# EnterpriseCV-6/Season-NeRF

Measured on AMD Instinct MI355X. Metric: ray-samples/sec (4096 rays x 96 samples forward render, T_NeRF 8x256), higher is better.
Workload: dtype i8x3 (16-bit fixed point as two int8 digits on v_mfma_i32_32x32x32_i8, exact int32 accumulate, fp32 epilogue)

## Files before the change

season_nerf_amd/csrc/kernels_i8x2.hip:

```cpp
#include "mlp_i8_device.h"

namespace snerf {

constexpr int NW2 = 8;
constexpr int TILE2 = 32 * NW2;
constexpr int PIECES2 = kChunkBytes / kFragBytes / NW2;
constexpr int RING2_D = 7;
#ifndef SNERF_PFX
#define SNERF_PFX 2
#endif
constexpr int PFX = SNERF_PFX;
static_assert(PIECES2 == 2 && kChunkPairs == 8, "the DMA below moves two pieces per wave; barrier positions assume 8-pair chunks");

#ifdef SNERF_STAMP
__device__ unsigned long long g_stamps[8 * 64];
__device__ __forceinline__ void stamp(int wave, int lane, int slot, bool on) {
    if (on && lane == 0) g_stamps[wave * 64 + slot] = __builtin_amdgcn_s_memtime();
}
#define STAMP(slot) stamp(wave, lane, slot, stamp_on)
#else
#define STAMP(slot)
#endif

struct Ring2 {
    uint32_t wr;
    uint32_t goff;
    uint32_t cur;
};
__device__ __forceinline__ uint32_t ring2_next(uint32_t off) {
    off += kChunkBytes;
    return off == RING2_D * kChunkBytes ? 0u : off;
}
__device__ __forceinline__ void dma_chunk2(const uint8_t* stream, uint32_t goff, lds_char* lds, uint32_t wr, int wave, int lane);
__device__ __forceinline__ void dma_chunk4(const uint8_t* stream, uint32_t goff, lds_char* lds, uint32_t wr, int wave, int lane);
#ifndef SNERF_X2_ALL_LOAD
#define SNERF_X2_OLD_LOADS 1
#endif
template <int PHASE>
__device__ __forceinline__ void ring_step2(Ring2& rg, const uint8_t* stream, uint32_t stream_bytes, lds_char* lds, int wave, int lane) {
#if defined(SNERF_ABLATE) && (ABL & 4)
    return;
#endif
#if defined(SNERF_X2_OLD_LOADS) && !defined(SNERF_STAMP)
    if (PHASE == 0) {
        asm volatile("s_waitcnt vmcnt(%0)\n\ts_barrier" ::"n"((RING2_D - 3) * 4) : "memory");
        dma_chunk4(stream, rg.goff, lds, rg.wr, wave, lane);
    } else {
        asm volatile("s_barrier" ::: "memory");
    }
    rg.goff += kChunkBytes;
    if (rg.goff >= stream_bytes) rg.goff = 0;
    rg.wr = ring2_next(rg.wr);
    return;
#endif
#ifdef SNERF_STAMP
    const unsigned long long t0_ = __builtin_amdgcn_s_memtime();
    asm volatile("s_waitcnt vmcnt(%0)" ::"n"((RING2_D - 3) * PIECES2) : "memory");
    const unsigned long long t1_ = __builtin_amdgcn_s_memtime();
    asm volatile("s_barrier" ::: "memory");
    const unsigned long long t2_ = __builtin_amdgcn_s_memtime();
    if (blockIdx.x == 0 && lane == 0) { g_stamps[wave * 64 + 62] += t1_ - t0_; g_stamps[wave * 64 + 63] += t2_ - t1_; }
#else
    asm volatile("s_waitcnt vmcnt(%0)\n\ts_barrier" ::"n"((RING2_D - 3) * PIECES2) : "memory");
#endif
    dma_chunk2(stream, rg.goff, lds, rg.wr, wave, lane);
    rg.goff += kChunkBytes;
    if (rg.goff >= stream_bytes) rg.goff = 0;
    rg.wr = ring2_next(rg.wr);
}
__device__ __forceinline__ void dma_chunk2(const uint8_t* stream, uint32_t goff, lds_char* lds, uint32_t wr, int wave, int lane) {
    const uint8_t* b0 = stream + goff + wave * (PIECES2 * kFragBytes);
    const uint32_t dst = (uint32_t)(uintptr_t)(lds + wr + wave * (PIECES2 * kFragBytes));
    const uint32_t voff = lane * 16;
    uint32_t keep;
    asm volatile(
        "s_mov_b32 %0, m0\n\t"
        "s_mov_b32 m0, %2\n\t"
        "s_nop 0\n\t"
        "global_load_lds_dwordx4 %1, %3\n\t"
        "s_add_u32 m0, m0, 0x400\n\t"
        "s_nop 0\n\t"
        "global_load_lds_dwordx4 %1, %4\n\t"
        "s_mov_b32 m0, %0"
        : "=&s"(keep)
        : "v"(voff), "s"(dst), "s"(b0), "s"(b0 + kFragBytes)
        : "memory", "scc");
}

__device__ __forceinline__ void dma_chunk4(const uint8_t* stream, uint32_t goff, lds_char* lds, uint32_t wr, int wave, int lane) {
    const uint8_t* b0 = stream + goff + wave * (4 * kFragBytes);
    const uint32_t dst = (uint32_t)(uintptr_t)(lds + wr + wave * (4 * kFragBytes));
    const uint32_t voff = lane * 16;
    uint32_t keep;
    asm volatile(
        "s_mov_b32 %0, m0\n\t"
        "s_mov_b32 m0, %2\n\t"
        "s_nop 0\n\t"
        "global_load_lds_dwordx4 %1, %3\n\t"
        "s_add_u32 m0, m0, 0x400\n\t"
        "s_nop 0\n\t"
        "global_load_lds_dwordx4 %1, %4\n\t"
        "s_add_u32 m0, m0, 0x400\n\t"
        "s_nop 0\n\t"
        "global_load_lds_dwordx4 %1, %5\n\t"
        "s_add_u32 m0, m0, 0x400\n\t"
        "s_nop 0\n\t"
        "global_load_lds_dwordx4 %1, %6\n\t"
        "s_mov_b32 m0, %0"
        : "=&s"(keep)
        : "v"(voff), "s"(dst), "s"(b0), "s"(b0 + kFragBytes), "s"(b0 + 2 * kFragBytes), "s"(b0 + 3 * kFragBytes)
        : "memory", "scc");
}

struct TabQ {
    f32x4 sc, bi;
};
__device__ __forceinline__ TabQ load_tab_quad(lds_cfloat* tab_l, int b, int h, int g) {
    typedef volatile const __attribute__((address_space(3))) f32x4 lds_vf32x4;
    lds_vf32x4* tp = (lds_vf32x4*)(tab_l + (b * 2 + h) * 32);
    TabQ t;
    t.sc = tp[g];
    t.bi = tp[4 + g];
    return t;
}
__device__ __forceinline__ TabQ load_tab_quad_h(lds_cfloat* tab_h, int b, int g) {
    typedef volatile const __attribute__((address_space(3))) f32x4 lds_vf32x4;
    lds_vf32x4* tp = (lds_vf32x4*)(tab_h + b * 64);
    TabQ t;
    t.sc = tp[g];
    t.bi = tp[4 + g];
    return t;
}
template <int NB, int KS0, int KS1, bool SIN, bool RAWL = false, int PHASE = 0, bool OPQ = false>
__device__ __forceinline__ void run_layer8x2(Ring2& rg, const uint8_t* stream, uint32_t stream_bytes, lds_char* lds, lds_cfloat* tab_l,
                                             const Frag8* in0, const Frag8* in1, Frag8* out, f32x16* raw, int wave, int lane,
                                             const float* rawx = nullptr) {
    constexpr int KS = KS0 + KS1, NP = NB * KS;
    typedef volatile const __attribute__((address_space(3))) f32x4 lds_vf32x4;
    f32x4 rq[4][3];
    const int h = lane >> 5;
    lds_cfloat* raw_l = tab_l + 2 * 32 * NB;
    lds_cfloat* tab_h = tab_l + 32 * h;
    lds_cfloat* raw_h = raw_l + 48 * h;
    if constexpr (OPQ) asm volatile("" : "+v"(tab_h), "+v"(raw_h));
    auto tabq = [&](int b_, int g_) { return OPQ ? load_tab_quad_h(tab_h, b_, g_) : load_tab_quad(tab_l, b_, h, g_); };
    i32x4 fT[PFX], fL[PFX];
#if defined(SNERF_ABLATE) && (ABL & 2)
    constexpr bool ABL2_ = true;
#pragma unroll
    for (int q = 0; q < PFX; ++q) { fT[q] = i32x4{lane, 1, 2, 3}; fL[q] = i32x4{4, lane, 6, 7}; }
#else
    constexpr bool ABL2_ = false;
#endif
#define REQUEST(QN, SLOT)                                                                              \
    do {                                                                                               \
        if ((QN) % kChunkPairs == 0) {                                                                 \
            ring_step2<PHASE>(rg, stream, stream_bytes, lds, wave, lane);                                \
            if ((QN) > 0) rg.cur = ring2_next(rg.cur);                                                 \
        }                                                                                              \
        lds_char* ap_ = lds + rg.cur + ((QN) % kChunkPairs) * kPairBytes + lane * 16;                  \
        if (!ABL2_) {                                                                                  \
            fT[SLOT] = *(lds_ci32x4*)ap_;                                                              \
            fL[SLOT] = *(lds_ci32x4*)(ap_ + kFragBytes);                                               \
        } else {                                                                                       \
            asm volatile("" : "+v"(fT[SLOT]), "+v"(fL[SLOT]));                                         \
        }                                                                                              \
    } while (0)
#pragma unroll
    for (int q = 0; q < PFX; ++q) {
        if (q < NP) REQUEST(q, q);
    }
    Acc8 acc;
    int m[16];
    TabQ tq[4];
    auto load_rq = [&](int g, int b_of) {
        if constexpr (RAWL) {
            lds_vf32x4* tp = OPQ ? (lds_vf32x4*)(raw_h + (b_of * 8 + g) * 12) : (lds_vf32x4*)(raw_l + ((b_of * 2 + h) * 4 + g) * 12);
            rq[g][0] = tp[0]; rq[g][1] = tp[1]; rq[g][2] = tp[2];
        }
    };
    auto quad = [&](int g, int b_of, const TabQ& t) {
        float v[4];
#pragma unroll
        for (int j = 0; j < 4; ++j) v[j] = __builtin_fmaf((float)m[4 * g + j], t.sc[j], t.bi[j]);
        if constexpr (RAWL) {
#pragma unroll
            for (int j = 0; j < 4; ++j)
                v[j] = __builtin_fmaf(rq[g][0][j], rawx[0], __builtin_fmaf(rq[g][1][j], rawx[1], __builtin_fmaf(rq[g][2][j], rawx[2], v[j])));
        }
        if (SIN) {
            int hi, lo;
            digits4(sin2pi(v[0]), sin2pi(v[1]), sin2pi(v[2]), sin2pi(v[3]), hi, lo);
            asm volatile("" : "+v"(hi), "+v"(lo));
            out[b_of].hi[g] = hi;
            out[b_of].lo[g] = lo;
        } else {
#pragma unroll
            for (int j = 0; j < 4; ++j) (*raw)[4 * g + j] = v[j];
        }
    };
#pragma unroll
    for (int b = 0; b < NB; ++b) {
        if (b > 0) {
            tq[0] = tabq(b - 1, 0);
            load_rq(0, b - 1);
#pragma unroll
            for (int i = 0; i < 16; ++i) m[i] = (int)(((uint32_t)acc.M[i] << 8) + (uint32_t)acc.X[i]);
            asm volatile("" ::: "memory");
            __builtin_amdgcn_sched_barrier(0);
        }
#pragma unroll
        for (int i = 0; i < 16; ++i) { acc.M[i] = 0; acc.X[i] = 0; }
#pragma unroll
        for (int s = 0; s < KS; ++s) {
            const int q = b * KS + s;
            const i32x4 aT = fT[q % PFX], aL = fL[q % PFX];
#ifndef SNERF_X2_NOPRIO
            if (((s + PHASE) & 1) == 0) __builtin_amdgcn_s_setprio(0); else __builtin_amdgcn_s_setprio(3);
#endif
            if (q + PFX < NP) REQUEST(q + PFX, q % PFX);
            if (b > 0) {
#pragma unroll
                for (int g = 1; g < 4; ++g) {
                    const int sg = (g * KS) / 4, lg = sg > 0 ? sg - 1 : 0;
                    if (lg == s) { tq[g] = tabq(b - 1, g); load_rq(g, b - 1); }
                }
            }
            mfma_i8x3(aT, aL, s < KS0 ? in0[s] : in1[s - KS0], acc);
            if (b > 0) {
#pragma unroll
                for (int g = 0; g < 4; ++g)
                    if ((g * KS) / 4 == s) quad(g, b - 1, tq[g]);
            }
            asm volatile("" ::: "memory");
#ifdef SNERF_X2_GROUPS
#pragma unroll
            for (int mm = 0; mm < 3; ++mm) {
                __builtin_amdgcn_sched_group_barrier(0x008, 1, 0);
                __builtin_amdgcn_sched_group_barrier(0x100, 1, 0);
                __builtin_amdgcn_sched_group_barrier(0x400, 2, 0);
                __builtin_amdgcn_sched_group_barrier(0x002, SNERF_X2_GROUPS, 0);
            }
#endif
            __builtin_amdgcn_sched_barrier(0);
        }
    }
#pragma unroll
    for (int i = 0; i < 16; ++i) m[i] = (int)(((uint32_t)acc.M[i] << 8) + (uint32_t)acc.X[i]);
#pragma unroll
    for (int g = 0; g < 4; ++g) {
        asm volatile("" ::: "memory");
        const TabQ t = tabq(NB - 1, g);
        load_rq(g, NB - 1);
        quad(g, NB - 1, t);
        asm volatile("" ::: "memory");
        __builtin_amdgcn_sched_barrier(0);
    }
    rg.cur = ring2_next(rg.cur);
#undef REQUEST
}

template <int W, int VARIANT, int PHASE>
__device__ __forceinline__ void field_tiles2(const MlpArgs& A, Ring2& rg, lds_char* lds, __attribute__((address_space(3))) float* tab_lds,
                                             int wave, int lane);

template <int W, int VARIANT>
__global__ __launch_bounds__(64 * NW2, 1) void mlp_i8x2_kernel(const MlpArgs A) {
    extern __shared__ __attribute__((aligned(16))) char smem[];
    constexpr int C_MAX = kMaxClasses;
    constexpr int W2 = W / 2;
    lds_char* lds = (lds_char*)smem;
    __attribute__((address_space(3))) float* tab_lds = (__attribute__((address_space(3))) float*)(lds + RING2_D * kChunkBytes);

    const int lane = threadIdx.x & 63;
    const int wave = __builtin_amdgcn_readfirstlane(threadIdx.x >> 6);
    const int h = lane >> 5;
    const int C = A.n_classes;

    for (int i = threadIdx.x; i < A.bias_floats; i += 64 * NW2) tab_lds[i] = A.bias[i];

    Ring2 rg;
    rg.cur = 0;
    rg.goff = 0;
    {
        uint32_t wr = 0;
#pragma unroll
        for (int c = 0; c < RING2_D - 2; ++c) {
#if defined(SNERF_X2_OLD_LOADS) && !defined(SNERF_STAMP)
            if (wave < 4) dma_chunk4(A.stream, rg.goff, lds, wr, wave, lane);
#else
            dma_chunk2(A.stream, rg.goff, lds, wr, wave, lane);
#endif
            rg.goff += kChunkBytes;
            if (rg.goff >= A.stream_bytes) rg.goff = 0;
            wr += kChunkBytes;
        }
        rg.wr = wr;
    }
    __syncthreads();

    if (wave < 4) field_tiles2<W, VARIANT, 0>(A, rg, lds, tab_lds, wave, lane);
    else field_tiles2<W, VARIANT, 1>(A, rg, lds, tab_lds, wave, lane);
    asm volatile("s_waitcnt vmcnt(0)" ::: "memory");
}

template <int W, int VARIANT, int PHASE>
__device__ __forceinline__ void field_tiles2(const MlpArgs& A, Ring2& rg, lds_char* lds, __attribute__((address_space(3))) float* tab_lds,
                                             int wave, int lane) {
    constexpr int C_MAX = kMaxClasses;
    constexpr int W2 = W / 2;
    const int h = lane >> 5;
    const int C = A.n_classes;
    const int64_t n_tiles = VARIANT == 3 ? (A.n + NW2 - 1) / NW2 : (A.n + TILE2 - 1) / TILE2;
    const int passes = VARIANT == 3 ? (A.n_samples + 31) / 32 : 1;
    int pass = 0;
    RaySum rs;
    for (int64_t tile = blockIdx.x; tile < n_tiles;) {
        const int64_t n = tile * TILE2 + wave * 32 + (lane & 31);
        const bool valid = n < A.n;
        const int64_t nc = valid ? n : A.n - 1;
        const int64_t g = VARIANT == 3 ? 0 : nc / A.group_size;

        float x0, x1, x2;
        if constexpr (VARIANT == 3) {
            raysum_point(rs, A, tile, NW2, wave, pass, lane, x0, x1, x2);
        } else if (A.points) {
            x0 = A.points[nc * 3]; x1 = A.points[nc * 3 + 1]; x2 = A.points[nc * 3 + 2];
        } else {
            const int64_t r = nc / A.n_samples;
            const int s = (int)(nc - r * A.n_samples);
            const float t = A.tvals[s], omt = __fsub_rn(1.f, t);
            x0 = __fadd_rn(__fmul_rn(A.top[r * 3], omt), __fmul_rn(A.bot[r * 3], t));
            x1 = __fadd_rn(__fmul_rn(A.top[r * 3 + 1], omt), __fmul_rn(A.bot[r * 3 + 1], t));
            x2 = __fadd_rn(__fmul_rn(A.top[r * 3 + 2], omt), __fmul_rn(A.bot[r * 3 + 2], t));
        }
        float s0 = 0.f, s1 = 0.f, s2 = 0.f;
        float pcls[C_MAX];
#pragma unroll
        for (int c = 0; c < C_MAX; ++c) pcls[c] = 0.f;
        if constexpr (VARIANT <= 1) { s0 = A.sun[g * 3]; s1 = A.sun[g * 3 + 1]; s2 = A.sun[g * 3 + 2]; }
        if constexpr (VARIANT == 0) {
            if (A.classes) {
#pragma unroll
                for (int c = 0; c < C_MAX; ++c) if (c < C) pcls[c] = A.classes[g * C + c];
            }
        }
#ifdef SNERF_STAMP
        const bool stamp_on = blockIdx.x == 0 && tile == (int64_t)blockIdx.x + gridDim.x;
#endif
        STAMP(0);
        Frag8 pe[PEPOS_KS8];
        make_pe_pos8<VARIANT == 3>(x0, x1, x2, h, pe);
        STAMP(1);

        constexpr int KW = W / 32, KW2 = W2 / 32;
        Frag8 hA[KW], hB[KW];
        f32x16 raw;
#define LAYER(L, NBv, K0, K1, SINv, IN0, IN1, OUT, RAW)                                                                       \
    run_layer8x2<NBv, K0, K1, SINv, false, PHASE, VARIANT == 3>(rg, A.stream, A.stream_bytes, lds, tab_lds + prog_table_start(PROG_FIELD, W, C_MAX, L), \
                                                  IN0, IN1, OUT, RAW, wave, lane)
#define LAYER_RAW(L, NBv, K0, K1, IN0, IN1, OUT, RX)                                                                          \
    run_layer8x2<NBv, K0, K1, true, true, PHASE, VARIANT == 3>(rg, A.stream, A.stream_bytes, lds, tab_lds + prog_table_start(PROG_FIELD, W, C_MAX, L), \
                                                 IN0, IN1, OUT, nullptr, wave, lane, RX)
        const float rx_p[3] = {x0, x1, x2}, rx_s[3] = {s0, s1, s2};
        LAYER_RAW(F_FC1, W / 32, PEPOS_KS8, 0, pe, nullptr, hA, rx_p); STAMP(2);
        LAYER(F_FC2, W / 32, KW, 0, true, hA, nullptr, hB, nullptr); STAMP(3);
        LAYER(F_FC3, W / 32, KW, 0, true, hB, nullptr, hA, nullptr); STAMP(4);
        LAYER(F_FC4, W / 32, KW, 0, true, hA, nullptr, hB, nullptr); STAMP(5);
        LAYER_RAW(F_FC5, W / 32, KW, PEPOS_KS8, hB, pe, hA, rx_p); STAMP(6);
        LAYER(F_FC6, W / 32, KW, 0, true, hA, nullptr, hB, nullptr); STAMP(7);
        LAYER(F_FC7, W / 32, KW, 0, true, hB, nullptr, hA, nullptr); STAMP(8);
        LAYER(F_FC8, W / 32, KW, 0, true, hA, nullptr, hB, nullptr); STAMP(9);
        Frag8 x1f[KW2];
        LAYER(F_FC9, W2 / 32, KW, 0, true, hB, nullptr, x1f, nullptr); STAMP(10);
        LAYER(F_HEAD, 1, KW2, 0, false, x1f, nullptr, nullptr, &raw); STAMP(11);
        const float col_r = raw[0], col_g = raw[1], col_b = raw[2], rho_raw = raw[3];
        float sv_raw = 0.f;
        float adj[3 * C_MAX];
#pragma unroll
        for (int i = 0; i < 3 * C_MAX; ++i) adj[i] = 0.f;
        if constexpr (VARIANT <= 1) {
            Frag8 ps[PESUN_KS8];
            make_pe_sun8(s0, s1, s2, h, ps);
            Frag8 sA[KW2], sB[KW2];
            LAYER_RAW(F_S1, W2 / 32, KW2, PESUN_KS8, x1f, ps, sA, rx_s); STAMP(12);
            LAYER(F_S2, W2 / 32, KW2, 0, true, sA, nullptr, sB, nullptr); STAMP(13);
            LAYER(F_S3, W2 / 32, KW2, 0, true, sB, nullptr, sA, nullptr); STAMP(14);
            LAYER(F_S4, 1, KW2, 0, false, sA, nullptr, nullptr, &raw); STAMP(15);
            sv_raw = raw[0];
        }
        if constexpr (VARIANT == 0) {
            LAYER(F_A1, W / 32, KW2, 0, true, x1f, nullptr, hA, nullptr); STAMP(16);
            LAYER(F_A2, W / 32, KW, 0, true, hA, nullptr, hB, nullptr); STAMP(17);
            LAYER(F_A3, W / 32, KW, 0, true, hB, nullptr, hA, nullptr); STAMP(18);
            LAYER(F_AC, 1, KW, 0, false, hA, nullptr, nullptr, &raw); STAMP(19);
#pragma unroll
            for (int i = 0; i < 3 * C_MAX; ++i) adj[i] = raw[i];
        }
#undef LAYER
#undef LAYER_RAW
        if constexpr (VARIANT == 3) {
            raysum_add(rs, A, tile, NW2, wave, pass, lane, rho_raw, x0, x1, x2);
            if (++pass == passes || raysum_saturated(rs, A, tile * NW2 + wave, wave, NW2, lane, (__attribute__((address_space(3))) float*)(tab_lds + A.bias_floats))) {
                raysum_end(rs, A, tile, NW2, wave, lane);
                pass = 0;
                tile += gridDim.x;
            }
        } else {
            if (h == 0 && valid) store_field_outputs<VARIANT>(A.out, n, C, x0, x1, x2, col_r, col_g, col_b, rho_raw, sv_raw, adj, pcls);
            tile += gridDim.x;
        }
        STAMP(20);
    }
    __builtin_amdgcn_s_setprio(0);
}

template <int W, int VARIANT>
static hipError_t launch_mlp_i8x2_t(const MlpArgs& a, int n_cu, hipStream_t st) {
    const int lds_bytes = RING2_D * kChunkBytes + a.bias_floats * 4 + kVoteBytes;
    const int64_t n_tiles = VARIANT == 3 ? (a.n + NW2 - 1) / NW2 : (a.n + TILE2 - 1) / TILE2;
    int grid = (int)(n_tiles < n_cu ? n_tiles : n_cu);
    if (grid < 1) grid = 1;
    auto k = mlp_i8x2_kernel<W, VARIANT>;
    hipError_t e = hipFuncSetAttribute((const void*)k, hipFuncAttributeMaxDynamicSharedMemorySize, lds_bytes);
    if (e != hipSuccess) return e;
    hipLaunchKernelGGL(k, dim3(grid), dim3(64 * NW2), lds_bytes, st, a);
    return hipGetLastError();
}

hipError_t launch_mlp_i8x2(int W, int variant, const MlpArgs& a, int n_cu, hipStream_t st) {
#define CASE(Wv)                                                              \
    if (W == Wv) {                                                            \
        if (variant == 0) return launch_mlp_i8x2_t<Wv, 0>(a, n_cu, st);       \
        if (variant == 1) return launch_mlp_i8x2_t<Wv, 1>(a, n_cu, st);       \
        if (variant == 3) return launch_mlp_i8x2_t<Wv, 3>(a, n_cu, st);       \
        return launch_mlp_i8x2_t<Wv, 2>(a, n_cu, st);                         \
    }
    CASE(64)
    CASE(256)
#undef CASE
    return hipErrorInvalidValue;
}

}

#ifdef SNERF_STAMP
extern "C" int snerf_debug_stamps(unsigned long long* host, int n) {
    if (n > 8 * 64) n = 8 * 64;
    hipError_t e = hipMemcpyFromSymbol(host, HIP_SYMBOL(snerf::g_stamps), (size_t)n * 8);
    unsigned long long zero[8 * 64] = {};
    (void)hipMemcpyToSymbol(HIP_SYMBOL(snerf::g_stamps), zero, sizeof(zero));
    return e == hipSuccess ? 0 : -3;
}
#endif
```

season_nerf_amd/csrc/pack.cpp:

```cpp
#include <atomic>
#include <cstdlib>
#include <mutex>
#include <thread>
#include "pack.h"

#include <cmath>
#include <cstring>

namespace snerf {

template <class F>
static bool parallel_layers(int L, std::string* err, F fn) {
    static const int cap = [] {
        const char* e = getenv("SNERF_PACK_THREADS");
        const unsigned hw = std::thread::hardware_concurrency();
        const int c = e ? atoi(e) : (int)(hw ? (hw < 8 ? hw : 8) : 1);
        return c < 1 ? 1 : c;
    }();
    const int T = cap < L ? cap : L;
    std::atomic<int> next{0};
    std::atomic<bool> ok{true};
    std::mutex mu;
    auto work = [&]() {
        for (;;) {
            const int l = next.fetch_add(1);
            if (l >= L || !ok.load()) break;
            std::string e;
            bool good = false;
            try {
                good = fn(l, &e);
            } catch (const std::exception& ex) {
                e = std::string("packing layer ") + std::to_string(l) + ": " + ex.what();
            } catch (...) {
                e = "packing layer " + std::to_string(l) + ": unknown exception";
            }
            if (!good) {
                std::lock_guard<std::mutex> g(mu);
                if (ok.exchange(false)) *err = e;
            }
        }
    };
    std::vector<std::thread> th;
    for (int t = 1; t < T; ++t) th.emplace_back(work);
    work();
    for (auto& t : th) t.join();
    return ok.load();
}

static inline uint16_t bf16_rne(float f) {
    uint32_t u;
    std::memcpy(&u, &f, 4);
    if ((u & 0x7f800000u) == 0x7f800000u) return (uint16_t)(u >> 16);
    u += 0x7fffu + ((u >> 16) & 1u);
    return (uint16_t)(u >> 16);
}
static inline float bf16_to_f32(uint16_t b) {
    uint32_t u = (uint32_t)b << 16;
    float f;
    std::memcpy(&f, &u, 4);
    return f;
}

const Tensor* Weights::find(const std::string& k) const {
    auto it = t.find(k);
    return it == t.end() ? nullptr : &it->second;
}

struct Src {
    const char* prefix;
    bool sine;
};

static const char* field_prefix(int l) {
    static const char* p[F_NUM] = {
        "G_NeRF_net.fc1", "G_NeRF_net.fc2", "G_NeRF_net.fc3", "G_NeRF_net.fc4", "G_NeRF_net.fc5", "G_NeRF_net.fc6",
        "G_NeRF_net.fc7", "G_NeRF_net.fc8", "G_NeRF_net.fc9", nullptr ,
        "G_NeRF_net.fc_solar_1", "G_NeRF_net.fc_solar_2", "G_NeRF_net.fc_solar_3", "G_NeRF_net.fc_solar_4",
        "adjust_layer_1", "adjust_layer_2", "adjust_layer_3", "adjust_col"};
    return p[l];
}
static const char* group_prefix(int l) {
    static const char* p[G_NUM] = {"time_layer_1", "time_layer_2", "get_class_layer", "G_NeRF_net.fc_sky_color_1",
                                   "G_NeRF_net.fc_sky_color_2"};
    return p[l];
}

struct Dense {
    int n = 0, k = 0;
    std::vector<double> W, b;
};

static bool fetch(const Weights& w, const std::string& key, size_t numel, const float** out, std::string* err) {
    const Tensor* t = w.find(key);
    if (!t) { *err = "missing tensor: " + key; return false; }
    if (t->data.size() != numel) {
        *err = "tensor " + key + " has " + std::to_string(t->data.size()) + " elements, expected " + std::to_string(numel);
        return false;
    }
    *out = t->data.data();
    return true;
}

static bool dense_sine(const Weights& w, const std::string& pre, int n, int k, bool fold_bn, Dense* d, std::string* err) {
    const float *W, *b;
    if (!fetch(w, pre + ".linear.weight", (size_t)n * k, &W, err)) return false;
    if (!fetch(w, pre + ".linear.bias", (size_t)n, &b, err)) return false;
    const bool has_bn = w.find(pre + ".norm.weight") != nullptr;
    const float *g = nullptr, *beta = nullptr, *mu = nullptr, *var = nullptr;
    if (has_bn) {
        if (!fold_bn) { *err = "layer " + pre + " has BatchNorm; only the folded (eval-mode) program is packed"; return false; }
        if (!fetch(w, pre + ".norm.weight", n, &g, err) || !fetch(w, pre + ".norm.bias", n, &beta, err) ||
            !fetch(w, pre + ".norm.running_mean", n, &mu, err) || !fetch(w, pre + ".norm.running_var", n, &var, err))
            return false;
    }
    const double inv2pi = 1.0 / (2.0 * M_PI);
    d->n = n; d->k = k;
    d->W.assign((size_t)n * k, 0.0); d->b.assign(n, 0.0);
    for (int r = 0; r < n; ++r) {
        double a = 1.0, shift = 0.0, off = 0.0;
        if (has_bn) { a = (double)g[r] / std::sqrt((double)var[r] + 1e-5); shift = mu[r]; off = beta[r]; }
        for (int c = 0; c < k; ++c) d->W[(size_t)r * k + c] = a * 30.0 * (double)W[(size_t)r * k + c] * inv2pi;
        d->b[r] = (a * (30.0 * (double)b[r] - shift) + off) * inv2pi;
    }
    return true;
}

static bool dense_linear(const Weights& w, const std::string& pre, int n, int k, Dense* d, std::string* err) {
    const float *W, *b;
    if (!fetch(w, pre + ".weight", (size_t)n * k, &W, err)) return false;
    if (!fetch(w, pre + ".bias", (size_t)n, &b, err)) return false;
    d->n = n; d->k = k;
    d->W.assign(W, W + (size_t)n * k);
    d->b.assign(b, b + n);
    return true;
}

static int ref_row(const LayerShape& s, int n) {
    const int b = n / 32, r = n % 32;
    switch (s.row_map) {
        case ROWS_ID: return n < s.n_ref ? n : -1;
        case ROWS_HEAD: return (b == 0 && r < 4) ? r : -1;
        case ROWS_SV: case ROWS_SKY: return (b == 0 && r < s.n_ref) ? r : -1;
        case ROWS_ADJ: case ROWS_CLASS:
            if (b != 0) return -1;
            for (int i = 0; i < s.n_ref && i < 16; ++i) if (acc_row(i, 0) == r) return i;
            return -1;
    }
    return -1;
}

static bool dense_layer(const Weights& w, int prog, int W, int C, int l, bool fold_bn, Dense* dp, std::string* err) {
    Dense& d = *dp;
    const LayerShape s = prog_layer(prog, W, C, l);
    const int k_ref = kind_features(s.kind0, s.ks0) + kind_features(s.kind1, s.ks1);
    if (prog == PROG_FIELD && l == F_HEAD) {
        Dense c3, s1;
        if (!dense_linear(w, "G_NeRF_net.fc10Col", 3, k_ref, &c3, err)) return false;
        if (!dense_linear(w, "G_NeRF_net.fc10Sigma", 1, k_ref, &s1, err)) return false;
        d.n = 4; d.k = k_ref; d.W = c3.W; d.b = c3.b;
        d.W.insert(d.W.end(), s1.W.begin(), s1.W.end()); d.b.push_back(s1.b[0]);
    } else {
        const std::string pre = prog == PROG_FIELD ? field_prefix(l) : group_prefix(l);
        int kr = k_ref;
        if (prog == PROG_GROUP && l == G_K2) kr = W / 4;
        if (s.out_kind == OUT_SIN) { if (!dense_sine(w, pre, s.n_ref, kr, fold_bn, &d, err)) return false; }
        else { if (!dense_linear(w, pre, s.n_ref, kr, &d, err)) return false; }
    }
    return true;
}

bool pack_program(const Weights& w, int prog, int W, int C, bool fold_bn, Packed* out, std::string* err) {
    if (W < 64 || W % 64 != 0) { *err = "layer width must be a multiple of 64 (got " + std::to_string(W) + ")"; return false; }
    if (C < 1 || C > kMaxClasses) { *err = "n_classes must be in [1," + std::to_string(kMaxClasses) + "]"; return false; }
    const int L = prog_layers(prog);
    out->stream.assign((size_t)prog_chunks(prog, W, C) * kChunkBytes, 0);
    out->bias.assign((size_t)prog_bias_floats(prog, W, C), 0.f);
    return parallel_layers(L, err, [&](int l, std::string* err) {
        const LayerShape s = prog_layer(prog, W, C, l);
        Dense d;
        if (!dense_layer(w, prog, W, C, l, fold_bn, &d, err)) return false;
        float* bias = out->bias.data() + prog_bias_start(prog, W, C, l);
        for (int b = 0; b < s.nb(); ++b)
            for (int h = 0; h < 2; ++h)
                for (int i = 0; i < 16; ++i) {
                    const int rr = ref_row(s, 32 * b + acc_row(i, h));
                    bias[b * 32 + h * 16 + i] = rr >= 0 ? (float)d.b[rr] : 0.f;
                }
        uint8_t* base = out->stream.data() + (size_t)prog_chunk_start(prog, W, C, l) * kChunkBytes;
        const int f0 = kind_features(s.kind0, s.ks0);
        for (int b = 0; b < s.nb(); ++b)
            for (int ks = 0; ks < s.ks(); ++ks) {
                uint16_t* hi = (uint16_t*)(base + (size_t)(b * s.ks() + ks) * kPairBytes);
                uint16_t* lo = hi + kFragBytes / 2;
                for (int lane = 0; lane < 64; ++lane) {
                    const int r = lane & 31, h = lane >> 5;
                    const int rr = ref_row(s, 32 * b + r);
                    for (int j = 0; j < 8; ++j) {
                        double v = 0.0;
                        if (rr >= 0) {
                            int col = -1;
                            if (ks < s.ks0) { const int f = slot_feature(s.kind0, 16 * ks + 8 * h + j); if (f >= 0) col = f; }
                            else { const int f = slot_feature(s.kind1, 16 * (ks - s.ks0) + 8 * h + j); if (f >= 0) col = f0 + f; }
                            if (col >= 0 && col < d.k) v = d.W[(size_t)rr * d.k + col];
                        }
                        const float vf = (float)v;
                        const uint16_t vh = bf16_rne(vf);
                        hi[lane * 8 + j] = vh;
                        lo[lane * 8 + j] = bf16_rne((float)(v - (double)bf16_to_f32(vh)));
                    }
                }
            }
        return true;
    });
}

bool permute_program_ks(const Packed& canon, int W, int C, Packed* out, std::string* err, int prog) {
    if (W % 256 != 0) { *err = "the K-split kernels need a width that is a multiple of 256 (got " + std::to_string(W) + ")"; return false; }
    if (canon.stream.size() != (size_t)prog_chunks(prog, W, C) * kChunkBytes) { *err = "permute_program_ks: not a packed program of this kind and width"; return false; }
    const int L = prog_layers(prog);
    auto start = [&](int l) { return prog == PROG_FIELD ? ks_chunk_start(W, C, l) : ks_chunk_start_g(W, C, l); };
    out->bias = canon.bias;
    out->stream.assign((size_t)start(L) * kChunkBytes, 0);
    for (int l = 0; l < L; ++l) {
        const LayerShape s = prog_layer(prog, W, C, l);
        const uint8_t* src = canon.stream.data() + (size_t)prog_chunk_start(prog, W, C, l) * kChunkBytes;
        uint8_t* dst = out->stream.data() + (size_t)start(l) * kChunkBytes;
        const int np = ks_layer_pairs(s);
        for (int a = 0; a < 2; ++a)
            for (int q = 0; q < np; ++q) {
                const int sp = ks_pair_source(s, a, q), b = sp / 4096, ks = sp % 4096;
                std::memcpy(dst + (size_t)(q / kKsParPairs) * kChunkBytes + (size_t)a * kKsParPairs * kPairBytes + (size_t)(q % kKsParPairs) * kPairBytes,
                            src + (size_t)(b * s.ks() + ks) * kPairBytes, kPairBytes);
            }
    }
    return true;
}

bool pack_program_i8(const Weights& w, int prog, int W, int C, bool fold_bn, Packed* out, std::string* err) {
    if (W < 64 || W % 64 != 0) { *err = "layer width must be a multiple of 64 (got " + std::to_string(W) + ")"; return false; }
    if (C < 1 || C > kMaxClasses) { *err = "n_classes must be in [1," + std::to_string(kMaxClasses) + "]"; return false; }
    const int L = prog_layers(prog);
    out->stream.assign((size_t)prog_chunks(prog, W, C, FMT_I8) * kChunkBytes, 0);
    out->bias.assign((size_t)prog_table_floats(prog, W, C), 0.f);
    return parallel_layers(L, err, [&](int l, std::string* err) {
        const LayerShape s = prog_layer(prog, W, C, l, FMT_I8);
        Dense d;
        if (!dense_layer(w, prog, W, C, l, fold_bn, &d, err)) return false;
        const int f0 = kind_features(s.kind0, s.ks0, FMT_I8);
        auto column = [&](int ks, int h, int j) {
            int col = -1;
            if (ks < s.ks0) { const int f = slot_feature8(s.kind0, ks, h, j); if (f >= 0) col = f; }
            else { const int f = slot_feature8(s.kind1, ks - s.ks0, h, j); if (f >= 0) col = f0 + f; }
            return (col >= 0 && col < d.k) ? col : -1;
        };
        const int rk = raw_kind(s), rdims = raw_dims(rk), rbase = (rk != IN_NONE && rk == s.kind1 && rk != s.kind0) ? f0 : 0;
        auto is_raw_col = [&](int c) { return rk != IN_NONE && c >= rbase && c < rbase + rdims; };
        const int n_pad = s.n_out;
        std::vector<double> scale(n_pad, 0.0);
        std::vector<long long> wsum(n_pad, 0);
        std::vector<int> wq((size_t)n_pad * d.k, 0);
        for (int n = 0; n < n_pad; ++n) {
            const int rr = ref_row(s, n);
            if (rr < 0) continue;
            double mx = 0.0;
            for (int c = 0; c < d.k; ++c) if (!is_raw_col(c)) mx = std::fmax(mx, std::fabs(d.W[(size_t)rr * d.k + c]));
            const double sn = mx > 0.0 ? mx / 32512.0 : 1.0;
            scale[n] = sn;
            for (int c = 0; c < d.k; ++c) wq[(size_t)n * d.k + c] = (int)std::llround(d.W[(size_t)rr * d.k + c] / sn);
        }
        uint8_t* base = out->stream.data() + (size_t)prog_chunk_start(prog, W, C, l, FMT_I8) * kChunkBytes;
        for (int b = 0; b < s.nb(); ++b)
            for (int ks = 0; ks < s.ks(); ++ks) {
                int8_t* Tf = (int8_t*)(base + (size_t)(b * s.ks() + ks) * kPairBytes);
                int8_t* Lf = Tf + kFragBytes;
                for (int lane = 0; lane < 64; ++lane) {
                    const int r = lane & 31, h = lane >> 5, n = 32 * b + r;
                    for (int j = 0; j < 16; ++j) {
                        const int col = column(ks, h, j);
                        int q = 0;
                        if (col >= 0 && ref_row(s, n) >= 0) { q = wq[(size_t)n * d.k + col]; wsum[n] += q; }
                        const int T = (q + 128) >> 8;
                        Tf[lane * 16 + j] = (int8_t)T;
                        Lf[lane * 16 + j] = (int8_t)(q - 256 * T);
                    }
                }
            }
        float* tab = out->bias.data() + prog_table_start(prog, W, C, l);
        for (int b = 0; b < s.nb(); ++b)
            for (int h = 0; h < 2; ++h)
                for (int i = 0; i < 16; ++i) {
                    const int n = 32 * b + acc_row(i, h), rr = ref_row(s, n);
                    float* t = tab + (b * 2 + h) * 32;
                    t[i] = rr >= 0 ? (float)(256.0 * scale[n] / 32767.0) : 0.f;
                    t[16 + i] = rr >= 0 ? (float)(d.b[rr] + 128.0 * scale[n] * (double)wsum[n] / 32767.0) : 0.f;
                }
        if (rk != IN_NONE) {
            float* rt = tab + 2 * s.n_out;
            for (int b = 0; b < s.nb(); ++b)
                for (int h = 0; h < 2; ++h)
                    for (int i = 0; i < 16; ++i) {
                        const int n = 32 * b + acc_row(i, h), rr = ref_row(s, n);
                        for (int dd = 0; dd < 3; ++dd)
                            rt[(((b * 2 + h) * 4 + i / 4) * 3 + dd) * 4 + i % 4] =
                                (rr >= 0 && dd < rdims && rbase + dd < d.k) ? (float)d.W[(size_t)rr * d.k + rbase + dd] : 0.f;
                    }
        }
        return true;
    });
}

static int hidden_source(int prog, int l) {
    if (prog == PROG_FIELD) {
        switch (l) {
            case F_FC1: return -1;
            case F_HEAD: case F_S1: case F_A1: return F_FC9;
            default: return l - 1;
        }
    }
    return (l == G_T1 || l == G_K1) ? -1 : l - 1;
}

static bool estimate_program(const Weights& w, int prog, int W, int C, std::vector<std::vector<double>>* out_var, double* hidden_rms,
                             long long* acc_bound, std::string* err) {
    const int L = prog_layers(prog);
    out_var->assign(L, {});
    const double qa = 1.0 / (12.0 * 32767.0 * 32767.0);
    const double lb = 5461.5 / (32767.0 * 32767.0);
    std::vector<Dense> dense(L);
    std::vector<std::vector<double>> own(L);
    std::vector<long long> bound_l(L, 0);
    std::vector<int> n_hidden_l(L, 0);
    if (!parallel_layers(L, err, [&](int l, std::string* err) {
            const LayerShape s = prog_layer(prog, W, C, l, FMT_I8);
            Dense& d = dense[l];
            if (!dense_layer(w, prog, W, C, l, true, &d, err)) return false;
            const int f0 = kind_features(s.kind0, s.ks0, FMT_I8);
            const int rk = raw_kind(s), rdims = raw_dims(rk), rbase = (rk != IN_NONE && rk == s.kind1 && rk != s.kind0) ? f0 : 0;
            auto is_raw_col = [&](int c) { return rk != IN_NONE && c >= rbase && c < rbase + rdims; };
            n_hidden_l[l] = s.kind0 == IN_H ? (f0 < d.k ? f0 : d.k) : 0;
            own[l].assign(d.n, 0.0);
            for (int n = 0; n < d.n; ++n) {
                const double* row = d.W.data() + (size_t)n * d.k;
                double mx = 0.0;
                for (int c = 0; c < d.k; ++c) if (!is_raw_col(c)) mx = std::fmax(mx, std::fabs(row[c]));
                const double sn = mx > 0.0 ? mx / 32512.0 : 1.0;
                double v = 0.0;
                long long sT = 0, sL = 0;
                for (int c = 0; c < d.k; ++c) {
                    if (is_raw_col(c)) continue;
                    const long long q = std::llround(row[c] / sn);
                    const long long T = (q + 128) >> 8, Lq = q - 256 * T;
                    sT += T < 0 ? -T : T; sL += Lq < 0 ? -Lq : Lq;
                    const double dw = row[c] - sn * (double)q;
                    v += 0.5 * dw * dw
                       + row[c] * row[c] * qa
                       + sn * sn * (double)(Lq * Lq) * lb;
                }
                const long long bound = 256LL * 128LL * sT + 128LL * (sT + sL);
                if (bound > bound_l[l]) bound_l[l] = bound;
                own[l][n] = v;
            }
            return true;
        }))
        return false;
    for (int l = 0; l < L; ++l) {
        const LayerShape s = prog_layer(prog, W, C, l, FMT_I8);
        const Dense& d = dense[l];
        const int f0 = kind_features(s.kind0, s.ks0, FMT_I8);
        const int rk = raw_kind(s), rdims = raw_dims(rk), rbase = (rk != IN_NONE && rk == s.kind1 && rk != s.kind0) ? f0 : 0;
        auto is_raw_col = [&](int c) { return rk != IN_NONE && c >= rbase && c < rbase + rdims; };
        const int src = hidden_source(prog, l);
        const std::vector<double>* ein = src >= 0 ? &(*out_var)[src] : nullptr;
        const int nh = ein ? (n_hidden_l[l] < (int)ein->size() ? n_hidden_l[l] : (int)ein->size()) : 0;
        std::vector<double>& ev = (*out_var)[l];
        ev.assign(d.n, 0.0);
        double sum = 0.0;
        if (bound_l[l] > *acc_bound) *acc_bound = bound_l[l];
        for (int n = 0; n < d.n; ++n) {
            const double* row = d.W.data() + (size_t)n * d.k;
            double v = own[l][n];
            for (int c = 0; c < nh; ++c)
                if (!is_raw_col(c)) v += row[c] * row[c] * (*ein)[c];
            ev[n] = s.out_kind == OUT_SIN ? (2.0 * M_PI) * (2.0 * M_PI) * 0.5 * v : v;
            sum += ev[n];
        }
        if (s.out_kind == OUT_SIN && d.n > 0) *hidden_rms = std::fmax(*hidden_rms, std::sqrt(sum / d.n));
    }
    return true;
}

bool estimate_i8(const Weights& w, int W, int C, I8Estimate* out, std::string* err) {
    if (W < 64 || W % 64 != 0) { *err = "layer width must be a multiple of 64 (got " + std::to_string(W) + ")"; return false; }
    if (C < 1 || C > kMaxClasses) { *err = "n_classes must be in [1," + std::to_string(kMaxClasses) + "]"; return false; }
    *out = I8Estimate();
    std::vector<std::vector<double>> ev;
    if (!estimate_program(w, PROG_FIELD, W, C, &ev, &out->hidden_rms, &out->acc_bound, err)) return false;
    auto rms = [](const std::vector<double>& v, int a, int b) {
        double s = 0.0;
        for (int i = a; i < b && i < (int)v.size(); ++i) s += v[i];
        return b > a ? std::sqrt(s / (b - a)) : 0.0;
    };
    out->head_rms[0] = rms(ev[F_HEAD], 3, 4);
    out->head_rms[1] = rms(ev[F_HEAD], 0, 3);
    out->head_rms[2] = rms(ev[F_S4], 0, 1);
    out->head_rms[3] = rms(ev[F_AC], 0, 3 * C);
    for (double v : out->head_rms) out->worst = std::fmax(out->worst, v);
    out->rgb_pred = 1.20 * out->head_rms[0] + 0.525 * out->head_rms[1] + 0.69 * out->head_rms[3] + 0.345 * out->head_rms[2];
    return true;
}

}
```

Baseline: 489.8 million.

## Defer each layer's last-block epilogue into the next layer's MFMA stream

Moves the epilogue state (dequantise, sine, digit split) into an Epi8 object. The final output block of each layer is no longer finished serially after its MFMA loop. Instead it is carried as pending work and interleaved into the first block of the next layer's MFMAs, when that layer does not need the block early. This is meant to hide the serial epilogue tail between layers behind matrix work, at the cost of more live registers and more complex ordering constraints. It also drops the non-OPQ table path and changes pack.cpp error reporting to keep the lowest failing layer.

Result: no change. 495.5 million (median of 6 runs) (+1.2%).

```diff
diff --git a/season_nerf_amd/csrc/kernels_i8x2.hip b/season_nerf_amd/csrc/kernels_i8x2.hip
--- a/season_nerf_amd/csrc/kernels_i8x2.hip
+++ b/season_nerf_amd/csrc/kernels_i8x2.hip
@@ -115,14 +115,6 @@
 struct TabQ {
     f32x4 sc, bi;
 };
-__device__ __forceinline__ TabQ load_tab_quad(lds_cfloat* tab_l, int b, int h, int g) {
-    typedef volatile const __attribute__((address_space(3))) f32x4 lds_vf32x4;
-    lds_vf32x4* tp = (lds_vf32x4*)(tab_l + (b * 2 + h) * 32);
-    TabQ t;
-    t.sc = tp[g];
-    t.bi = tp[4 + g];
-    return t;
-}
 __device__ __forceinline__ TabQ load_tab_quad_h(lds_cfloat* tab_h, int b, int g) {
     typedef volatile const __attribute__((address_space(3))) f32x4 lds_vf32x4;
     lds_vf32x4* tp = (lds_vf32x4*)(tab_h + b * 64);
@@ -131,19 +123,94 @@
     t.bi = tp[4 + g];
     return t;
 }
-template <int NB, int KS0, int KS1, bool SIN, bool RAWL = false, int PHASE = 0, bool OPQ = false>
-__device__ __forceinline__ void run_layer8x2(Ring2& rg, const uint8_t* stream, uint32_t stream_bytes, lds_char* lds, lds_cfloat* tab_l,
-                                             const Frag8* in0, const Frag8* in1, Frag8* out, f32x16* raw, int wave, int lane,
-                                             const float* rawx = nullptr) {
-    constexpr int KS = KS0 + KS1, NP = NB * KS;
-    typedef volatile const __attribute__((address_space(3))) f32x4 lds_vf32x4;
+
+template <int NB_, bool SIN, bool RAWL = false>
+struct Epi8 {
+    static constexpr int NB = NB_;
+    static constexpr bool live = true;
+    lds_cfloat* tab_l;
+    lds_cfloat* tab_h;
+    lds_cfloat* raw_h;
+    Frag8* out;
+    f32x16* raw;
+    const float* rawx;
+    int h;
+    int m[16];
+    TabQ tq[4];
     f32x4 rq[4][3];
-    const int h = lane >> 5;
-    lds_cfloat* raw_l = tab_l + 2 * 32 * NB;
-    lds_cfloat* tab_h = tab_l + 32 * h;
-    lds_cfloat* raw_h = raw_l + 48 * h;
-    if constexpr (OPQ) asm volatile("" : "+v"(tab_h), "+v"(raw_h));
-    auto tabq = [&](int b_, int g_) { return OPQ ? load_tab_quad_h(tab_h, b_, g_) : load_tab_quad(tab_l, b_, h, g_); };
+
+    __device__ __forceinline__ void init(lds_cfloat* tab, Frag8* out_, f32x16* raw_, const float* rawx_, int lane) {
+        tab_l = tab;
+        out = out_;
+        raw = raw_;
+        rawx = rawx_;
+        h = lane >> 5;
+    }
+    __device__ __forceinline__ void bases() {
+        int hv = h;
+        asm volatile("" : "+v"(hv));
+        tab_h = tab_l + 32 * hv;
+        raw_h = tab_l + 2 * 32 * NB + 48 * hv;
+    }
+    __device__ __forceinline__ void merge(const Acc8& acc) {
+#pragma unroll
+        for (int i = 0; i < 16; ++i) m[i] = (int)(((uint32_t)acc.M[i] << 8) + (uint32_t)acc.X[i]);
+    }
+    __device__ __forceinline__ void load(int g, int b) {
+        typedef volatile const __attribute__((address_space(3))) f32x4 lds_vf32x4;
+        tq[g] = load_tab_quad_h(tab_h, b, g);
+        if constexpr (RAWL) {
+            lds_vf32x4* tp = (lds_vf32x4*)(raw_h + (b * 8 + g) * 12);
+            rq[g][0] = tp[0]; rq[g][1] = tp[1]; rq[g][2] = tp[2];
+        }
+    }
+    __device__ __forceinline__ void quad(int g, int b) {
+        float v[4];
+#pragma unroll
+        for (int j = 0; j < 4; ++j) v[j] = __builtin_fmaf((float)m[4 * g + j], tq[g].sc[j], tq[g].bi[j]);
+        if constexpr (RAWL) {
+#pragma unroll
+            for (int j = 0; j < 4; ++j)
+                v[j] = __builtin_fmaf(rq[g][0][j], rawx[0], __builtin_fmaf(rq[g][1][j], rawx[1], __builtin_fmaf(rq[g][2][j], rawx[2], v[j])));
+        }
+        if constexpr (SIN) {
+            int hi, lo;
+            digits4(sin2pi(v[0]), sin2pi(v[1]), sin2pi(v[2]), sin2pi(v[3]), hi, lo);
+            asm volatile("" : "+v"(hi), "+v"(lo));
+            out[b].hi[g] = hi;
+            out[b].lo[g] = lo;
+        } else {
+#pragma unroll
+            for (int j = 0; j < 4; ++j) (*raw)[4 * g + j] = v[j];
+        }
+    }
+    __device__ __forceinline__ void flush() {
+#pragma unroll
+        for (int g = 0; g < 4; ++g) {
+            asm volatile("" ::: "memory");
+            load(g, NB - 1);
+            quad(g, NB - 1);
+            asm volatile("" ::: "memory");
+            __builtin_amdgcn_sched_barrier(0);
+        }
+    }
+};
+struct NoEpi {
+    static constexpr int NB = 1;
+    static constexpr bool live = false;
+    __device__ __forceinline__ void load(int, int) {}
+    __device__ __forceinline__ void quad(int, int) {}
+    __device__ __forceinline__ void flush() {}
+};
+
+template <int KS0, int KS1, bool RD, int PHASE, class P, class E>
+__device__ __forceinline__ void run_layer8x2(Ring2& rg, const uint8_t* stream, uint32_t stream_bytes, lds_char* lds,
+                                             const Frag8* in0, const Frag8* in1, P& pend, E& ep, int wave, int lane) {
+    constexpr int NB = E::NB, KS = KS0 + KS1, NP = NB * KS;
+    constexpr int DEP = RD ? P::NB - 1 : KS;
+    constexpr int KSP = (3 * KS) / 4 < DEP ? KS : DEP;
+    static_assert(!RD || P::NB <= KS0, "the pending block is read through in0");
+    ep.bases();
     i32x4 fT[PFX], fL[PFX];
 #if defined(SNERF_ABLATE) && (ABL & 2)
     constexpr bool ABL2_ = true;
@@ -170,42 +237,23 @@
     for (int q = 0; q < PFX; ++q) {
         if (q < NP) REQUEST(q, q);
     }
+    if constexpr (P::live) {
+        if constexpr (KSP == 0) {
+            pend.flush();
+        } else {
+#pragma unroll
+            for (int g = 0; g < 4; ++g)
+                if ((g * KSP) / 4 == 0) pend.load(g, P::NB - 1);
+            asm volatile("" ::: "memory");
+            __builtin_amdgcn_sched_barrier(0);
+        }
+    }
     Acc8 acc;
-    int m[16];
-    TabQ tq[4];
-    auto load_rq = [&](int g, int b_of) {
-        if constexpr (RAWL) {
-            lds_vf32x4* tp = OPQ ? (lds_vf32x4*)(raw_h + (b_of * 8 + g) * 12) : (lds_vf32x4*)(raw_l + ((b_of * 2 + h) * 4 + g) * 12);
-            rq[g][0] = tp[0]; rq[g][1] = tp[1]; rq[g][2] = tp[2];
-        }
-    };
-    auto quad = [&](int g, int b_of, const TabQ& t) {
-        float v[4];
-#pragma unroll
-        for (int j = 0; j < 4; ++j) v[j] = __builtin_fmaf((float)m[4 * g + j], t.sc[j], t.bi[j]);
-        if constexpr (RAWL) {
-#pragma unroll
-            for (int j = 0; j < 4; ++j)
-                v[j] = __builtin_fmaf(rq[g][0][j], rawx[0], __builtin_fmaf(rq[g][1][j], rawx[1], __builtin_fmaf(rq[g][2][j], rawx[2], v[j])));
-        }
-        if (SIN) {
-            int hi, lo;
-            digits4(sin2pi(v[0]), sin2pi(v[1]), sin2pi(v[2]), sin2pi(v[3]), hi, lo);
-            asm volatile("" : "+v"(hi), "+v"(lo));
-            out[b_of].hi[g] = hi;
-            out[b_of].lo[g] = lo;
-        } else {
-#pragma unroll
-            for (int j = 0; j < 4; ++j) (*raw)[4 * g + j] = v[j];
-        }
-    };
 #pragma unroll
     for (int b = 0; b < NB; ++b) {
         if (b > 0) {
-            tq[0] = tabq(b - 1, 0);
-            load_rq(0, b - 1);
-#pragma unroll
-            for (int i = 0; i < 16; ++i) m[i] = (int)(((uint32_t)acc.M[i] << 8) + (uint32_t)acc.X[i]);
+            ep.load(0, b - 1);
+            ep.merge(acc);
             asm volatile("" ::: "memory");
             __builtin_amdgcn_sched_barrier(0);
         }
@@ -215,6 +263,7 @@
         for (int s = 0; s < KS; ++s) {
             const int q = b * KS + s;
             const i32x4 aT = fT[q % PFX], aL = fL[q % PFX];
+            constexpr bool PQ = P::live && KSP > 0;
 #ifndef SNERF_X2_NOPRIO
             if (((s + PHASE) & 1) == 0) __builtin_amdgcn_s_setprio(0); else __builtin_amdgcn_s_setprio(3);
 #endif
@@ -223,14 +272,24 @@
 #pragma unroll
                 for (int g = 1; g < 4; ++g) {
                     const int sg = (g * KS) / 4, lg = sg > 0 ? sg - 1 : 0;
-                    if (lg == s) { tq[g] = tabq(b - 1, g); load_rq(g, b - 1); }
+                    if (lg == s) ep.load(g, b - 1);
+                }
+            } else if (PQ) {
+#pragma unroll
+                for (int g = 1; g < 4; ++g) {
+                    const int sg = (g * KSP) / 4;
+                    if (sg > 0 && sg - 1 == s) pend.load(g, P::NB - 1);
                 }
             }
             mfma_i8x3(aT, aL, s < KS0 ? in0[s] : in1[s - KS0], acc);
             if (b > 0) {
 #pragma unroll
                 for (int g = 0; g < 4; ++g)
-                    if ((g * KS) / 4 == s) quad(g, b - 1, tq[g]);
+                    if ((g * KS) / 4 == s) ep.quad(g, b - 1);
+            } else if (PQ) {
+#pragma unroll
+                for (int g = 0; g < 4; ++g)
+                    if ((g * KSP) / 4 == s) pend.quad(g, P::NB - 1);
             }
             asm volatile("" ::: "memory");
 #ifdef SNERF_X2_GROUPS
@@ -245,17 +304,7 @@
             __builtin_amdgcn_sched_barrier(0);
         }
     }
-#pragma unroll
-    for (int i = 0; i < 16; ++i) m[i] = (int)(((uint32_t)acc.M[i] << 8) + (uint32_t)acc.X[i]);
-#pragma unroll
-    for (int g = 0; g < 4; ++g) {
-        asm volatile("" ::: "memory");
-        const TabQ t = tabq(NB - 1, g);
-        load_rq(g, NB - 1);
-        quad(g, NB - 1, t);
-        asm volatile("" ::: "memory");
-        __builtin_amdgcn_sched_barrier(0);
-    }
+    ep.merge(acc);
     rg.cur = ring2_next(rg.cur);
 #undef REQUEST
 }
@@ -355,26 +404,24 @@
 
         constexpr int KW = W / 32, KW2 = W2 / 32;
         Frag8 hA[KW], hB[KW];
-        f32x16 raw;
-#define LAYER(L, NBv, K0, K1, SINv, IN0, IN1, OUT, RAW)                                                                       \
-    run_layer8x2<NBv, K0, K1, SINv, false, PHASE, VARIANT == 3>(rg, A.stream, A.stream_bytes, lds, tab_lds + prog_table_start(PROG_FIELD, W, C_MAX, L), \
-                                                  IN0, IN1, OUT, RAW, wave, lane)
-#define LAYER_RAW(L, NBv, K0, K1, IN0, IN1, OUT, RX)                                                                          \
-    run_layer8x2<NBv, K0, K1, true, true, PHASE, VARIANT == 3>(rg, A.stream, A.stream_bytes, lds, tab_lds + prog_table_start(PROG_FIELD, W, C_MAX, L), \
-                                                 IN0, IN1, OUT, nullptr, wave, lane, RX)
+#define EPI(E, L, NBv, SINv, RAWLv, OUT, RAW, RX)                                                                              \
+    Epi8<NBv, SINv, RAWLv> E;                                                                                              \
+    E.init(tab_lds + prog_table_start(PROG_FIELD, W, C_MAX, L), OUT, RAW, RX, lane)
+#define LAYER(K0, K1, RD, IN0, IN1, PREV, E) run_layer8x2<K0, K1, RD, PHASE>(rg, A.stream, A.stream_bytes, lds, IN0, IN1, PREV, E, wave, lane)
         const float rx_p[3] = {x0, x1, x2}, rx_s[3] = {s0, s1, s2};
-        LAYER_RAW(F_FC1, W / 32, PEPOS_KS8, 0, pe, nullptr, hA, rx_p); STAMP(2);
-        LAYER(F_FC2, W / 32, KW, 0, true, hA, nullptr, hB, nullptr); STAMP(3);
-        LAYER(F_FC3, W / 32, KW, 0, true, hB, nullptr, hA, nullptr); STAMP(4);
-        LAYER(F_FC4, W / 32, KW, 0, true, hA, nullptr, hB, nullptr); STAMP(5);
-        LAYER_RAW(F_FC5, W / 32, KW, PEPOS_KS8, hB, pe, hA, rx_p); STAMP(6);
-        LAYER(F_FC6, W / 32, KW, 0, true, hA, nullptr, hB, nullptr); STAMP(7);
-        LAYER(F_FC7, W / 32, KW, 0, true, hB, nullptr, hA, nullptr); STAMP(8);
-        LAYER(F_FC8, W / 32, KW, 0, true, hA, nullptr, hB, nullptr); STAMP(9);
+        NoEpi e0;
+        EPI(e1, F_FC1, W / 32, true, true, hA, nullptr, rx_p);     LAYER(PEPOS_KS8, 0, false, pe, nullptr, e0, e1); STAMP(2);
+        EPI(e2, F_FC2, W / 32, true, false, hB, nullptr, nullptr); LAYER(KW, 0, true, hA, nullptr, e1, e2); STAMP(3);
+        EPI(e3, F_FC3, W / 32, true, false, hA, nullptr, nullptr); LAYER(KW, 0, true, hB, nullptr, e2, e3); STAMP(4);
+        EPI(e4, F_FC4, W / 32, true, false, hB, nullptr, nullptr); LAYER(KW, 0, true, hA, nullptr, e3, e4); STAMP(5);
+        EPI(e5, F_FC5, W / 32, true, true, hA, nullptr, rx_p);     LAYER(KW, PEPOS_KS8, true, hB, pe, e4, e5); STAMP(6);
+        EPI(e6, F_FC6, W / 32, true, false, hB, nullptr, nullptr); LAYER(KW, 0, true, hA, nullptr, e5, e6); STAMP(7);
+        EPI(e7, F_FC7, W / 32, true, false, hA, nullptr, nullptr); LAYER(KW, 0, true, hB, nullptr, e6, e7); STAMP(8);
+        EPI(e8, F_FC8, W / 32, true, false, hB, nullptr, nullptr); LAYER(KW, 0, true, hA, nullptr, e7, e8); STAMP(9);
         Frag8 x1f[KW2];
-        LAYER(F_FC9, W2 / 32, KW, 0, true, hB, nullptr, x1f, nullptr); STAMP(10);
-        LAYER(F_HEAD, 1, KW2, 0, false, x1f, nullptr, nullptr, &raw); STAMP(11);
-        const float col_r = raw[0], col_g = raw[1], col_b = raw[2], rho_raw = raw[3];
+        EPI(e9, F_FC9, W2 / 32, true, false, x1f, nullptr, nullptr); LAYER(KW, 0, true, hB, nullptr, e8, e9); STAMP(10);
+        f32x16 r_head, r_sun, r_adj;
+        EPI(eh, F_HEAD, 1, false, false, nullptr, &r_head, nullptr); LAYER(KW2, 0, true, x1f, nullptr, e9, eh); STAMP(11);
         float sv_raw = 0.f;
         float adj[3 * C_MAX];
 #pragma unroll
@@ -383,22 +430,28 @@
             Frag8 ps[PESUN_KS8];
             make_pe_sun8(s0, s1, s2, h, ps);
             Frag8 sA[KW2], sB[KW2];
-            LAYER_RAW(F_S1, W2 / 32, KW2, PESUN_KS8, x1f, ps, sA, rx_s); STAMP(12);
-            LAYER(F_S2, W2 / 32, KW2, 0, true, sA, nullptr, sB, nullptr); STAMP(13);
-            LAYER(F_S3, W2 / 32, KW2, 0, true, sB, nullptr, sA, nullptr); STAMP(14);
-            LAYER(F_S4, 1, KW2, 0, false, sA, nullptr, nullptr, &raw); STAMP(15);
-            sv_raw = raw[0];
-        }
-        if constexpr (VARIANT == 0) {
-            LAYER(F_A1, W / 32, KW2, 0, true, x1f, nullptr, hA, nullptr); STAMP(16);
-            LAYER(F_A2, W / 32, KW, 0, true, hA, nullptr, hB, nullptr); STAMP(17);
-            LAYER(F_A3, W / 32, KW, 0, true, hB, nullptr, hA, nullptr); STAMP(18);
-            LAYER(F_AC, 1, KW, 0, false, hA, nullptr, nullptr, &raw); STAMP(19);
-#pragma unroll
-            for (int i = 0; i < 3 * C_MAX; ++i) adj[i] = raw[i];
-        }
+            EPI(es1, F_S1, W2 / 32, true, true, sA, nullptr, rx_s);     LAYER(KW2, PESUN_KS8, false, x1f, ps, eh, es1); STAMP(12);
+            EPI(es2, F_S2, W2 / 32, true, false, sB, nullptr, nullptr); LAYER(KW2, 0, true, sA, nullptr, es1, es2); STAMP(13);
+            EPI(es3, F_S3, W2 / 32, true, false, sA, nullptr, nullptr); LAYER(KW2, 0, true, sB, nullptr, es2, es3); STAMP(14);
+            EPI(es4, F_S4, 1, false, false, nullptr, &r_sun, nullptr);  LAYER(KW2, 0, true, sA, nullptr, es3, es4); STAMP(15);
+            if constexpr (VARIANT == 0) {
+                EPI(ea1, F_A1, W / 32, true, false, hA, nullptr, nullptr); LAYER(KW2, 0, false, x1f, nullptr, es4, ea1); STAMP(16);
+                EPI(ea2, F_A2, W / 32, true, false, hB, nullptr, nullptr); LAYER(KW, 0, true, hA, nullptr, ea1, ea2); STAMP(17);
+                EPI(ea3, F_A3, W / 32, true, false, hA, nullptr, nullptr); LAYER(KW, 0, true, hB, nullptr, ea2, ea3); STAMP(18);
+                EPI(eac, F_AC, 1, false, false, nullptr, &r_adj, nullptr); LAYER(KW, 0, true, hA, nullptr, ea3, eac); STAMP(19);
+                eac.flush();
+#pragma unroll
+                for (int i = 0; i < 3 * C_MAX; ++i) adj[i] = r_adj[i];
+            } else {
+                es4.flush();
+            }
+            sv_raw = r_sun[0];
+        } else {
+            eh.flush();
+        }
+        const float col_r = r_head[0], col_g = r_head[1], col_b = r_head[2], rho_raw = r_head[3];
+#undef EPI
 #undef LAYER
-#undef LAYER_RAW
         if constexpr (VARIANT == 3) {
             raysum_add(rs, A, tile, NW2, wave, pass, lane, rho_raw, x0, x1, x2);
             if (++pass == passes || raysum_saturated(rs, A, tile * NW2 + wave, wave, NW2, lane, (__attribute__((address_space(3))) float*)(tab_lds + A.bias_floats))) {
diff --git a/season_nerf_amd/csrc/pack.cpp b/season_nerf_amd/csrc/pack.cpp
--- a/season_nerf_amd/csrc/pack.cpp
+++ b/season_nerf_amd/csrc/pack.cpp
@@ -19,12 +19,12 @@
     }();
     const int T = cap < L ? cap : L;
     std::atomic<int> next{0};
-    std::atomic<bool> ok{true};
+    std::atomic<int> first_bad{L};
     std::mutex mu;
     auto work = [&]() {
         for (;;) {
             const int l = next.fetch_add(1);
-            if (l >= L || !ok.load()) break;
+            if (l >= L || l > first_bad.load()) break;
             std::string e;
             bool good = false;
             try {
@@ -36,7 +36,10 @@
             }
             if (!good) {
                 std::lock_guard<std::mutex> g(mu);
-                if (ok.exchange(false)) *err = e;
+                if (l < first_bad.load()) {
+                    first_bad.store(l);
+                    *err = e;
+                }
             }
         }
     };
@@ -44,7 +47,7 @@
     for (int t = 1; t < T; ++t) th.emplace_back(work);
     work();
     for (auto& t : th) t.join();
-    return ok.load();
+    return first_bad.load() == L;
 }
 
 static inline uint16_t bf16_rne(float f) {
```
